# caidj0/Raytracer-2025

Hardware: AMD Instinct MI355X
Metric: Msamples/s (pixels x traced spp / s), book-1 random spheres 1920x1080, 512 spp (484 traced) (higher is better)
Workload: dtype f64

## Files before the change

### include/rt_mi355x.h

```cpp
#ifndef RT_MI355X_H
#define RT_MI355X_H

#include <stddef.h>
#include <stdint.h>

#ifdef __cplusplus
extern "C" {
#endif

#define RT_ABI_VERSION 3

enum rt_status {
    RT_OK = 0,
    RT_EINVAL = -1,
    RT_EHANDLE = -2,
    RT_EMOVED = -3,
    RT_EDEGENERATE = -4,
    RT_EPANIC = -5,
    RT_EUNSUPPORTED = -6,
    RT_EDEVICE = -7,
    RT_ENOMEM = -8,
    RT_ESTACK = -9
};

// ... 243 lines not shown
int32_t rt_render_gather_mode(const rt_scene* s);

int32_t rt_render_partials_get(rt_scene* s, double* out, uint64_t n_values);

int32_t rt_render_primary_get(rt_scene* s, uint16_t* out, uint64_t n_values);

int32_t rt_math_selftest(int32_t fn, int32_t impl, const double* a, const double* b, double* out, uint64_t n);

int32_t rt_walk_selftest(int32_t fn, const double* in, double* out, uint64_t n);

int32_t rt_disney_selftest(int32_t fn, const rt_disney_params* params, const double base_color[3], const double* in,
                           double* out, uint64_t n);

int32_t rt_bvh_selftest(rt_scene* s, int32_t list);
int32_t rt_world_selftest(rt_scene* s, int32_t world, int32_t lights, int32_t background_tex);

#define RT_COMM_ID_BYTES 128
int32_t rt_comm_unique_id(uint8_t id[RT_COMM_ID_BYTES]);
rt_comm* rt_comm_init(const uint8_t id[RT_COMM_ID_BYTES], int32_t nranks, int32_t rank);
void rt_comm_destroy(rt_comm* comm);

int32_t rt_to_rgb_device(const float* linear_device, uint8_t* srgb_device, uint64_t n_values, int32_t toon_map,
                         void* stream);
int32_t rt_write_png(const char* path, uint32_t width, uint32_t height, const uint8_t* rgb);
int32_t rt_camera_from_json(const char* path, rt_camera* cam);

#ifdef __cplusplus
}
#endif
#endif
// ... 1 lines not shown
```

### raytracer-2025_amd/capi.py

```python
import ctypes as C

c_double3 = C.c_double * 3
c_double4 = C.c_double * 4


class RtCamera(C.Structure):

    _fields_ = [
        ("aspect_ratio", C.c_double),
        ("image_width", C.c_uint32),
        ("samples_per_pixel", C.c_uint32),
        ("max_depth", C.c_uint32),
        ("background_tex", C.c_int32),
        ("vertical_fov_in_degrees", C.c_double),
        ("look_from", c_double3),
        ("look_at", c_double3),
        ("vec_up", c_double3),
        ("defocus_angle_in_degrees", C.c_double),
        ("focus_distance", C.c_double),
        ("toon_map", C.c_int32),
        ("reserved", C.c_int32),
    ]


# ... 227 lines not shown
    "shard_rows": (_U, [C.POINTER(RtCamera), C.POINTER(RtRenderOpts)]),
    "render_device": (_I, [_P, _I, _I, C.POINTER(RtCamera), C.POINTER(RtRenderOpts), _P]),
    "render_device_wait": (_I, [_P, C.POINTER(RtStats)]),
    "render_gather_mode": (_I, [_P]),
    "to_rgb_device": (_I, [_P, _P, C.c_uint64, _I, _P]),
    "write_png": (_I, [C.c_char_p, C.c_uint32, C.c_uint32, _P]),
    "camera_from_json": (_I, [C.c_char_p, C.POINTER(RtCamera)]),
    "world_info_get": (_I, [_P, _I, _I, _I, _U, C.POINTER(RtWorldInfo)]),
    "render_partials_get": (_I, [_P, _DP, C.c_uint64]),
    "render_primary_get": (_I, [_P, C.POINTER(C.c_uint16), C.c_uint64]),
    "math_selftest": (_I, [_I, _I, _DP, _DP, _DP, C.c_uint64]),
    "walk_selftest": (_I, [_I, _DP, _DP, C.c_uint64]),
    "disney_selftest": (_I, [_I, C.POINTER(RtDisneyParams), _DP, _DP, _DP, C.c_uint64]),
    "bvh_selftest": (_I, [_P, _I]),
    "world_selftest": (_I, [_P, _I, _I, _I]),
    "comm_unique_id": (_I, [C.POINTER(C.c_uint8)]),
    "comm_init": (_P, [C.POINTER(C.c_uint8), _I, _I]),
    "comm_destroy": (None, [_P]),
}

GPU_ONLY = ("world_hit", "world_hit_device", "world_occluded", "world_occluded_device", "radiance_opts_default", "world_radiance", "world_radiance_device", "lights_opts_default", "lights_pdf", "lights_pdf_device", "lights_sample", "lights_sample_device", "scatter_opts_default", "world_scatter", "world_scatter_device", "render_gather_mode", "render_partials_get", "render_primary_get", "math_selftest", "walk_selftest", "disney_params_default", "mat_disney", "mat_portal", "wavefront_load_flags", "disney_selftest", "bvh_selftest", "world_selftest", "comm_unique_id", "comm_init", "comm_destroy")

ORACLE_EXTRAS = {
    "render_partials": (_I, [_P, _I, _I, C.POINTER(RtCamera), C.POINTER(RtRenderOpts), _DP, C.POINTER(RtStats)]),
    "render_f64": (_I, [_P, _I, _I, C.POINTER(RtCamera), C.POINTER(RtRenderOpts), _DP, C.POINTER(C.c_uint8),
                        C.POINTER(RtStats), C.POINTER(C.c_uint64)]),
    "work_count_fields": (_U, []),
}

STATUS = {
    0: "RT_OK", -1: "RT_EINVAL", -2: "RT_EHANDLE", -3: "RT_EMOVED", -4: "RT_EDEGENERATE",
    -5: "RT_EPANIC", -6: "RT_EUNSUPPORTED", -7: "RT_EDEVICE", -8: "RT_ENOMEM", -9: "RT_ESTACK",
}


class RtError(RuntimeError):
# ... 37 lines not shown
```

### raytracer-2025_amd/csrc/rt_builds.h

```cpp
#pragma once
#include <hip/hip_runtime.h>

#include "rt_kernel.h"

namespace rtk {

struct Diag {
#ifdef RT_DIAG
    unsigned long long cyc_refill = 0, cyc_trace = 0, cyc_shade = 0, cyc_media = 0;
    unsigned long long cyc_miss = 0, cyc_queue = 0, cyc_draws = 0;
    unsigned long long wave_trace_iters = 0, lane_trace_iters = 0, node_visits = 0, sphere_tests = 0, main_iters = 0;
    unsigned long long load_cyc = 0, loads = 0;
    unsigned long long pops = 0, pop_reads = 0;
    unsigned long long big_tests = 0, big_hits = 0;
    unsigned long long u_steps = 0, u_uniform = 0, u_uniform_node = 0, u_active = 0, u_same = 0;
    unsigned long long u_top[4] = {0, 0, 0, 0}, l_top[4] = {0, 0, 0, 0}, l_node = 0;
    unsigned long long sh_rounds = 0, sh_lanes = 0, sh_classes = 0;
    unsigned long long pure_rounds = 0, pure_lanes = 0, pure_max_pn = 0;
    unsigned long long cls_rounds[11] = {}, cls_lanes[11] = {};
    unsigned long long cyc_camera = 0, prim_rays = 0, prim_tests = 0;
#endif
};
#ifdef RT_DIAG
constexpr int RT_DIAG_N = 64;
__device__ unsigned long long g_diag[RT_DIAG_N];
#define RT_DIAG_ONLY(x) x
#else
#define RT_DIAG_ONLY(x)
#endif
#ifdef RT_ISA_MARKS
#define RT_ISA_MARK(name) asm volatile(";@@phase " name)
#else
#define RT_ISA_MARK(name)
#endif

#ifdef RT_WAVE_TRACE
constexpr uint32_t RT_TRACE_LANES = 1u << 19, RT_TRACE_W = 12;
__device__ unsigned long long g_lane_trace[RT_TRACE_LANES * RT_TRACE_W];
constexpr uint32_t RT_HIST_N = 1024, RT_HIST_TICKS = 25000;
// ... 20 lines not shown
#ifdef RT_CHECK
constexpr uint32_t K_CHECK_SLAB = 15;
static_assert(K_CHECK_SLAB > K_POPXF, "the slab guard's marker must not be a ref kind");
constexpr uint32_t K_CHECK_PRIMARY = 14;
static_assert(K_CHECK_PRIMARY > K_POPXF, "the primary-ray guard's marker must not be a ref kind");
__device__ unsigned long long g_check[2];
__device__ __noinline__ void check_fail(uint32_t ref) {
    atomicAdd(&g_check[0], 1ull);
    atomicCAS(&g_check[1], 0ull, (1ull << 32) | ref);
}
#endif
__device__ __forceinline__ uint32_t ref_idx(const SceneView& S, uint32_t ref) {
    const uint32_t i = ref_index(ref);
#ifdef RT_CHECK
    const uint32_t k = ref_kind(ref);
    if (k != K_NONE && i >= S.n_ref[k]) {
        check_fail(ref);
        return 0u;
    }
#endif
    return i;
}
__device__ __forceinline__ void check_run(const SceneView& S, uint32_t first, uint32_t n) {
#ifdef RT_CHECK
    if (n && first + n > S.n_ref[K_QUAD]) check_fail(make_ref(K_QUAD, first + n - 1));
#endif
}

}
```

### raytracer-2025_amd/csrc/rt_kernel_hit.hip

```cpp
#include <hip/hip_runtime.h>

#include "../../include/rt_mi355x.h"
#include "rt_kernel.h"
#include "rt_math.h"
#include "rt_builds.h"
#include "rt_geom.h"
#include "rt_stack.h"
#include "rt_walk.h"
#include "rt_walk4.h"
#include "rt_record.h"

namespace rtk {

struct HitParams {
    SceneView S;
    const rt_ray* rays;
    rt_hit_record* out;
    uint64_t n;
    uint32_t key0, key1;
    RT_GLOBAL uint2* stack_ovf;
};

template <int TIER>
__global__ void __launch_bounds__(TIER == TIER_BASIC ? RT_BLOCK_BASIC : RT_BLOCK) rt_hit_kernel(const HitParams P) {
// ... 21 lines not shown
    for (uint64_t w0 = (uint64_t)blockIdx.x * BLK + (threadIdx.x & ~63u); w0 < P.n; w0 += stride) {
        const uint64_t i = w0 + (threadIdx.x & 63u);
        const bool live = i < P.n;
        Ray ray{};
        double t_max = 0.0;
        if (live) {
            const rt_ray q = P.rays[i];
            ray.o = d3(q.origin[0], q.origin[1], q.origin[2]);
            ray.d = d3(q.dir[0], q.dir[1], q.dir[2]);
            ray.time = q.time;
            t_max = q.t_max;
        }
        rng.pixel = (uint32_t)i;
        rng.begin(1);
        Trav<TIER> T;
        trace_begin<TIER>(S, ray, T);
        T.cl.set(t_max);
        if constexpr (B4) {
            if (!live) T.cur = 0u;
            bool walking = live;
            while (__ballot(walking))
                walking = trace4_step(S, ray, T, stk, pq, (const RT_LDS float4*)node_lds, dg);
        } else if (live) {
            while (trace_step<TIER>(S, ray, T, stk, rng, med, dg)) {
            }
            if constexpr (tier_full(TIER)) media_phase<TIER>(S, ray, T, stk, rng, med);
        }
        if (live) {
            rt_hit_record o{};
            o.mat = -1;
            if (T.found) {
                bool panic = false;
// ... 41 lines not shown
```

### raytracer-2025_amd/csrc/rt_kernel_occl.hip

```cpp
#include <hip/hip_runtime.h>

#include "../../include/rt_mi355x.h"
#include "rt_kernel.h"
#include "rt_math.h"
#include "rt_builds.h"
#include "rt_geom.h"
#include "rt_stack.h"
#include "rt_walk.h"
#include "rt_walk4.h"

namespace rtk {

struct OcclParams {
    SceneView S;
    const rt_ray* rays;
    uint8_t* out;
    uint64_t n;
    uint32_t key0, key1;
    RT_GLOBAL uint2* stack_ovf;
};

template <int TIER>
__global__ void __launch_bounds__(TIER == TIER_BASIC ? RT_BLOCK_BASIC : RT_BLOCK) rt_occl_kernel(const OcclParams P) {
    const SceneView& S = P.S;
// ... 20 lines not shown
    for (uint64_t w0 = (uint64_t)blockIdx.x * BLK + (threadIdx.x & ~63u); w0 < P.n; w0 += stride) {
        const uint64_t i = w0 + (threadIdx.x & 63u);
        const bool live = i < P.n;
        Ray ray{};
        double t_max = 0.0;
        if (live) {
            const rt_ray q = P.rays[i];
            ray.o = d3(q.origin[0], q.origin[1], q.origin[2]);
            ray.d = d3(q.dir[0], q.dir[1], q.dir[2]);
            ray.time = q.time;
            t_max = q.t_max;
        }
        rng.pixel = (uint32_t)i;
        rng.begin(1);
        Trav<TIER> T;
        trace_begin<TIER>(S, ray, T);
        T.cl.set(t_max);
        if constexpr (B4) {
            if (!live) T.cur = 0u;
            bool walking = live;
            while (__ballot(walking)) {
                walking = trace4_step(S, ray, T, stk, pq, (const RT_LDS float4*)node_lds, dg);
                if (T.found) {
                    T.cur = 0u;
                    T.sp = 0;
                    T.pn = 0;
                    walking = false;
                }
            }
        } else if (live) {
            while (!T.found && trace_step<TIER>(S, ray, T, stk, rng, med, dg)) {
            }
            if constexpr (tier_full(TIER)) {
                if (!T.found) media_phase<TIER>(S, ray, T, stk, rng, med);
            }
// ... 31 lines not shown
```

### raytracer-2025_amd/csrc/rt_kernel_path.hip

```cpp
#include <hip/hip_runtime.h>

#include "../../include/rt_mi355x.h"
#include "rt_kernel.h"
#include "rt_math.h"
#include "rt_slab.h"
#include "rt_primary.h"
#include "rt_plan.h"
#include "rt_queue.h"
#include "rt_path_entry.h"
#include "rt_builds.h"
#include "rt_frame.h"
#include "rt_texture.h"
#include "rt_geom.h"
#include "rt_stack.h"
#include "rt_walk.h"
#include "rt_walk4.h"
#include "rt_record.h"
#include "rt_lights.h"
#include "rt_shade.h"

namespace rtk {

#ifndef RT_BASIC_WAVES
#define RT_BASIC_WAVES 4
// ... 196 lines not shown
                if (!walking) {
                    T.cl.c = __builtin_huge_val();
                    T.cl.c_f = __builtin_huge_valf();
                    T.sp = 0;
                    T.found = false;
                    T.pn = 0;
                    T.nxf = 0;
                    T.hit.nxf = 0;
                    T.nmed = 0;
                    const bool begin = !no_path && !pmiss;
                    T.cur = begin ? bword(S, S.world_root) : 0u;
                    if (begin) {
                        rng.begin(vertex);
                        ++n_rays;
                        walking = true;
                    }
                } else {
                    trace_unpark_state2(T, pk2);
                }
            } else if (!no_path && !walking) {
                rng.begin(vertex);
                ++n_rays;
                trace_begin<TIER>(S, ray, T);
                walking = true;
            }
            RT_DIAG_ONLY(const unsigned long long t_b0 = __builtin_amdgcn_s_memtime(); dg.cyc_refill += t_b0 - t_loop0;)
            RT_ISA_MARK("walk");
            auto step = [&]() -> bool {
                return trace4_step(S, ray, T, stk, pq, (const RT_LDS float4*)node_lds, dg);
            };
            if constexpr (BATCH >= 64) {
#ifdef RT_WAVE_TRACE
                while (walking) walking = step(), ++trace_steps;
#else
                while (walking) walking = step();
#endif
            } else {
                const unsigned long long active = __ballot(true);
// ... 363 lines not shown
    atomicAdd(&g_diag[20], dg.u_same);
    for (int k = 0; k < 4; ++k) {
        atomicAdd(&g_diag[24 + k], dg.u_top[k]);
        atomicAdd(&g_diag[28 + k], dg.l_top[k]);
    }
    atomicAdd(&g_diag[32], dg.l_node);
    atomicAdd(&g_diag[33], dg.sh_rounds);
    atomicAdd(&g_diag[34], dg.sh_lanes);
    atomicAdd(&g_diag[35], dg.sh_classes);
    atomicAdd(&g_diag[36], dg.pure_rounds);
    atomicAdd(&g_diag[37], dg.pure_lanes);
    atomicAdd(&g_diag[38], dg.pure_max_pn);
    if (lane == 0) atomicAdd(&g_diag[61], dg.cyc_camera);
    atomicAdd(&g_diag[62], dg.prim_rays);
    atomicAdd(&g_diag[63], dg.prim_tests);
    for (int k = 0; k < 11; ++k) {
        atomicAdd(&g_diag[39 + k], dg.cls_rounds[k]);
        atomicAdd(&g_diag[50 + k], dg.cls_lanes[k]);
    }
#endif
#ifdef RT_WAVE_TRACE
    hist.flush();
    if (trace_lane < RT_TRACE_LANES) {
        unsigned long long* t = g_lane_trace + (uint64_t)trace_lane * RT_TRACE_W;
        t[0] = trace_t0;
        t[1] = __builtin_amdgcn_s_memrealtime();
        t[2] = trace_items;
        t[3] = n_rays;
        t[4] = trace_tq;
        t[5] = trace_q;
// ... 149 lines not shown
```

### raytracer-2025_amd/csrc/rt_kernel_radiance.hip

```cpp
#include <hip/hip_runtime.h>

#include "../../include/rt_mi355x.h"
#include "rt_kernel.h"
#include "rt_math.h"
#include "rt_queue.h"
#include "rt_builds.h"
#include "rt_texture.h"
#include "rt_geom.h"
#include "rt_stack.h"
#include "rt_walk.h"
#include "rt_walk4.h"
#include "rt_record.h"
#include "rt_lights.h"
#include "rt_shade.h"

namespace rtk {

struct RadParams {
    SceneView S;
    const rt_ray* rays;
    rt_radiance* out;
    uint32_t n;
    uint32_t first_index;
    uint32_t samples, max_depth;
// ... 99 lines not shown
        double t_max = 0.0;
        const bool first_walk = !done && !in_path;
        if (first_walk) {
            const rt_ray q = P.rays[item];
            ray.o = d3(q.origin[0], q.origin[1], q.origin[2]);
            ray.d = d3(q.dir[0], q.dir[1], q.dir[2]);
            ray.time = q.time;
            t_max = q.t_max;
            rng.sample = s;
            beta = d3(1, 1, 1);
            L = d3(0, 0, 0);
            vertex = 1;
            in_path = true;
        }
        Trav<TIER> T;
        trace_begin<TIER>(S, ray, T);
        if (in_path) {
            rng.begin(vertex);
            if (first_walk) T.cl.set(t_max);
        }
        if constexpr (B4) {
            if (!in_path) T.cur = 0u;
            bool walking = in_path;
            while (__ballot(walking))
                walking = trace4_step(S, ray, T, stk, pq, (const RT_LDS float4*)node_lds, dg);
        } else {
            while (trace_step<TIER>(S, ray, T, stk, rng, med, dg)) {
            }
            if constexpr (tier_full(TIER)) media_phase<TIER>(S, ray, T, stk, rng, med);
        }
        if (!in_path) continue;
        bool panic = false;
        bool end_path;
        if constexpr (B4) {
// ... 94 lines not shown
```

### raytracer-2025_amd/csrc/rt_kernel_scatter.hip

```cpp
#include <hip/hip_runtime.h>

#include "../../include/rt_mi355x.h"
#include "rt_kernel.h"
#include "rt_math.h"
#include "rt_builds.h"
#include "rt_texture.h"
#include "rt_geom.h"
#include "rt_stack.h"
#include "rt_walk.h"
#include "rt_walk4.h"
#include "rt_record.h"
#include "rt_lights.h"
#include "rt_shade.h"
#include "rt_scatter.h"

namespace rtk {

struct ScatterParams {
    SceneView S;
    const rt_ray* rays;
    const double* eval_dirs;
    const uint32_t* indices;
    rt_scatter* out;
    uint64_t n;
// ... 51 lines not shown
        const uint64_t i = w0 + (threadIdx.x & 63u);
        const bool live = i < P.n;
        Ray ray{};
        double t_max = 0.0;
        rng.pixel = P.first_index + (uint32_t)i;
        if (live) {
            const rt_ray q = P.rays[i];
            ray.o = d3(q.origin[0], q.origin[1], q.origin[2]);
            ray.d = d3(q.dir[0], q.dir[1], q.dir[2]);
            ray.time = q.time;
            t_max = q.t_max;
            if (P.indices) rng.pixel = P.indices[i];
        }
        rng.begin(P.vertex);
        Trav<TIER> T;
        trace_begin<TIER>(S, ray, T);
        T.cl.set(t_max);
        if constexpr (B4) {
            if (!live) T.cur = 0u;
            bool walking = live;
            while (__ballot(walking))
                walking = trace4_step(S, ray, T, stk, pq, (const RT_LDS float4*)node_lds, dg);
        } else if (live) {
            while (trace_step<TIER>(S, ray, T, stk, rng, med, dg)) {
            }
            if constexpr (tier_full(TIER)) media_phase<TIER>(S, ray, T, stk, rng, med);
        }
        if (!live) continue;
        char* const rec_out = (char*)&P.out[i];
        {
            double v[10] = {0, 0, 0, 0, 0, 0, 0, 0, 0, 0};
            int32_t mat = -1;
// ... 71 lines not shown
```

### raytracer-2025_amd/csrc/rt_layout.h

```cpp
#pragma once
#include "rt_planar_filter.h"
#include <hip/hip_runtime.h>
#include <stdint.h>

#if defined(__HIP_DEVICE_COMPILE__)
#define RT_GLOBAL __attribute__((address_space(1)))
#define RT_LDS __attribute__((address_space(3)))
#else
#define RT_GLOBAL
#define RT_LDS
#endif

namespace rtk {

enum RefKind : uint32_t {
    K_NONE = 0,
    K_BVH = 1,
    K_LIST = 2,
    K_SPHERE = 3,
    K_MSPHERE = 4,
    K_QUAD = 5,
    K_TRI = 6,
    K_XFORM = 7,
    K_MEDIUM = 8,
    K_POPXF = 9,
};

__host__ __device__ inline uint32_t make_ref(uint32_t kind, uint32_t index) { return (kind << 28) | index; }
__host__ __device__ inline uint32_t ref_kind(uint32_t r) { return r >> 28; }
__host__ __device__ inline uint32_t ref_index(uint32_t r) { return r & 0x0FFFFFFFu; }
constexpr uint32_t REF_NONE = 0u;

struct alignas(16) DNodeSlot {
    union {
        struct {
            float lo[3], hi[3];
            uint32_t pad[2];
        } box;
        double sphere[4];
    };
};
struct alignas(16) DNode {
    DNodeSlot slot[2];
    uint32_t c0, c1;
    uint32_t pad[2];
};
// ... 137 lines not shown
    const RT_GLOBAL DXform* xforms;
    const RT_GLOBAL DMedium* media;
    const RT_GLOBAL DMaterial* materials;
    const RT_GLOBAL DTexture* textures;
    const RT_GLOBAL float* texels;
    const RT_GLOBAL DPerlin* perlin;
    uint32_t world_root;
    uint32_t lights_root;
    int32_t background_tex;
    int32_t bg_kind;
    double bg_c0[3], bg_c1[3];
    uint32_t stack_need;
    uint32_t features;
    uint32_t n_nodes4;
    uint32_t n_perlin;
    uint32_t n_ref[16];
};

enum : int32_t { BG_NONE = 0, BG_SKY = 1, BG_OTHER = 2 };

enum : uint32_t {
    F_XFORM = 1u,
    F_MEDIUM = 2u,
    F_PLANAR = 4u,
    F_MSPHERE = 8u,
    F_LIGHTS = 16u,
    F_TEXFULL = 32u,
    F_MATFULL = 64u,
    F_REMAP = 128u,
    F_GENERAL = 512u,
    F_NORMALMAP = 256u,
    F_DISNEY = 1024u,
// ... 5 lines not shown
```

### raytracer-2025_amd/csrc/rt_render.cpp

```cpp
#include <dlfcn.h>

#include <algorithm>
#include <chrono>
#include <cstdlib>
#include <cstring>
#include <memory>
#include <mutex>
#include <map>
#include <thread>

#include <rccl/rccl.h>

#include "../../include/rt_mi355x.h"
#include "rt_kernel.h"
#include "rt_primary.h"
#include "rt_scene.hpp"

namespace {
struct RcclApi {
    bool ok = false;
    std::string err;
    ncclResult_t (*get_unique_id)(ncclUniqueId*) = nullptr;
    ncclResult_t (*comm_init_rank)(ncclComm_t*, int, ncclUniqueId, int) = nullptr;
    ncclResult_t (*comm_init_all)(ncclComm_t*, int, const int*) = nullptr;
// ... 224 lines not shown
        bvh4_convert(hw, RT_STACK_BASIC, true, rtk::NODE_LDS_CAP, rtk::NODE_LDS_CAP_BATCH) > RT_STACK_BASIC)
        tier = rtk::TIER_MESH;
    if (tier == rtk::TIER_MESH && bvh4_convert(hw, RT_STACK_MAX, false) > RT_STACK_MAX) tier = rtk::TIER_FULL;
    if (tier == rtk::TIER_FULL && hw.nodes.empty()) return rtk::TIER_FULL_FLAT;
    if (rtk::tier_full_bvh(tier)) {
        const uint32_t need = bvh4_convert(hw, RT_STACK_MAX, false);
        if (need > RT_STACK_MAX) {
            set_error(RT_ESTACK, "world needs " + std::to_string(need) + " traversal-stack entries, kernel has " +
                                     std::to_string(RT_STACK_MAX));
            return -1;
        }
    }
    return tier;
}

static int32_t hip_fail(hipError_t e, const char* what) {
    return set_error(RT_EDEVICE, std::string(what) + ": " + hipGetErrorString(e));
}

template <class T>
static size_t put(std::vector<char>& blob, const std::vector<T>& v) {
    size_t off = (blob.size() + 255) & ~(size_t)255;
    blob.resize(off + v.size() * sizeof(T));
    if (!v.empty()) std::memcpy(blob.data() + off, v.data(), v.size() * sizeof(T));
    return off;
}

static void pack_world(const HostWorld& hw, std::vector<char>& blob, rtk::SceneView& v) {
    auto off = [](size_t o) { return (uintptr_t)o; };
    v.portals = (const rtk::DPortal*)off(put(blob, hw.portals));
// ... 41 lines not shown
static int32_t build_flat(rt_scene* s, int32_t world, int32_t lights, int32_t bg, bool reference_bvh, FlatWorld& fw) {
    std::lock_guard<std::mutex> lk(fw.m);
    if (fw.done) {
        if (fw.rc != RT_OK) set_error(fw.rc, fw.err);
        return fw.rc;
    }
    fw.done = true;
    auto t0 = std::chrono::steady_clock::now();
    HostWorld hw;
    int32_t rc = flatten(s, world, lights, bg, reference_bvh, hw);
    constexpr uint32_t MATERIAL_TIERS = rtk::F_DISNEY | rtk::F_PORTAL | rtk::F_GENERAL;
    fw.has_disney = rc == RT_OK && (hw.features & MATERIAL_TIERS) != 0;
    if (fw.for_query) hw.features &= ~MATERIAL_TIERS;
    int tier = rc == RT_OK ? prepare_tier(hw) : -1;
    if (rc == RT_OK && tier < 0) rc = RT_ESTACK;
#ifdef RT_CHECK
    if (rc == RT_OK && std::getenv("RT_CHECK_INJECT") && std::getenv("RT_CHECK_INJECT")[0] == '1') {
        for (rtk::DNode4& nd : hw.nodes4)
            for (int k = 0; k < 4; ++k) {
                const uint32_t kind = rtk::ref_kind(nd.ref[k]);
                const size_t n = kind == rtk::K_SPHERE ? hw.spheres.size()
                                 : (kind == rtk::K_QUAD || kind == rtk::K_TRI) ? hw.planars.size() : 0;
                if (n) nd.ref[k] = rtk::make_ref(kind, (uint32_t)n + rtk::ref_index(nd.ref[k]));
            }
    }
#endif
    if (rc == RT_OK) {
        const uint32_t stack_cap = rtk_stack_entries(tier);
        if (hw.stack_need > stack_cap)
            rc = set_error(RT_ESTACK, "world needs " + std::to_string(hw.stack_need) +
// ... 19 lines not shown
            for (int k = 0; k < 3; ++k) v.bg_c0[k] = t.color[k], v.bg_c1[k] = t.color2[k];
    }
    v.stack_need = hw.stack_need;
    v.features = hw.features;
    v.n_nodes4 = (uint32_t)hw.nodes4.size();
    v.n_perlin = (uint32_t)hw.perlin.size();
    std::memset(v.n_ref, 0, sizeof v.n_ref);
    v.n_ref[rtk::K_BVH] = (uint32_t)hw.nodes4.size();
    v.n_ref[rtk::K_LIST] = (uint32_t)hw.list_children.size();
    v.n_ref[rtk::K_SPHERE] = (uint32_t)hw.spheres.size();
    v.n_ref[rtk::K_MSPHERE] = (uint32_t)hw.msph_center.size();
    v.n_ref[rtk::K_QUAD] = v.n_ref[rtk::K_TRI] = (uint32_t)hw.planars.size();
    v.n_ref[rtk::K_XFORM] = (uint32_t)hw.xforms.size();
    v.n_ref[rtk::K_MEDIUM] = (uint32_t)hw.media.size();
    v.n_ref[rtk::K_POPXF] = 1;
    fw.tier = tier;
    fw.stack_need = hw.stack_need;
    fw.n_prims = hw.n_prims;
    fw.ms = std::chrono::duration<double, std::milli>(std::chrono::steady_clock::now() - t0).count();
    return RT_OK;
}

static int32_t slot_for(RenderState* r, size_t k, int device, DeviceWorld*& out) {
    DeviceWorld* d = r->slots[k];
    if (d && d->device != device) {
        destroy_device_world(d);
        r->slots[k] = d = nullptr;
        (void)hipSetDevice(device);
    }
    if (d) {
// ... 1078 lines not shown
    return lights_device(s, world, lights, opts, L_SAMPLE, origins3_dev, nullptr, n, out_dev);
}

int32_t rt_world_info_get(rt_scene* s, int32_t world, int32_t lights, int32_t bg, uint32_t flags, rt_world_info* out) {
    if (!s || !out) return set_error(RT_EINVAL, "null argument");
    if (world < 0 || (size_t)world >= s->objs.size() || s->objs[world].hidden)
        return set_error(RT_EHANDLE, "unknown world handle");
    try {
        HostWorld hw;
        int32_t rc = flatten(s, world, lights, bg, (flags & RT_FLAG_REFERENCE_BVH) != 0, hw);
        if (rc != RT_OK) return rc;
        out->primitives = (uint32_t)hw.n_prims;
        out->bvh_leaves = (uint32_t)hw.n_bvh_leaves;
        const int tier = prepare_tier(hw);
        if (tier < 0) return RT_ESTACK;
        std::vector<char> blob;
        rtk::SceneView view{};
        pack_world(hw, blob, view);
        out->device_bytes = blob.size();
        out->bvh_nodes = (uint32_t)hw.nodes4.size();
        out->stack_need = hw.stack_need;
        out->kernel_tier = (uint32_t)tier;
        out->features = hw.features;
        return RT_OK;
    } catch (const std::bad_alloc&) {
        return set_error(RT_ENOMEM, "out of host memory");
    }
}

int32_t rt_render_device_wait(rt_scene* s, rt_stats* st) {
    return wait(s, st);
}

int32_t rt_render_gather_mode(const rt_scene* s) {
    const RenderState* r = s ? s->rs : nullptr;
    if (!r || r->n_parts == 0) return set_error(RT_EINVAL, "nothing rendered on this scene");
    return r->gather_mode;
}

// ... 231 lines not shown
```

### raytracer-2025_amd/csrc/rt_scene.cpp

```cpp
#include "rt_kernel.h"
#include "rt_image.hpp"
#include "rt_scene.hpp"
#include "rt_slab.h"

#include <algorithm>
#include <cstring>
#include <exception>
#include <functional>
#include <limits>
#include <system_error>
#include <thread>
#include <unordered_map>

#include "../../include/rt_mi355x.h"

#ifndef RT_EXPAND_LEAF_LISTS
#define RT_EXPAND_LEAF_LISTS 1
#endif

namespace rth {

static thread_local std::string g_error;
int32_t set_error(int32_t code, const std::string& msg) {
    g_error = msg;
// ... 194 lines not shown
constexpr int MAX_XF_NESTING = 2;

#ifndef RT_SAH_SWEEP_MAX
#define RT_SAH_SWEEP_MAX 2048
#endif

struct Flattener {
    const rt_scene* s;
    HostWorld& out;
    bool reference_bvh;
    std::unordered_map<int, std::pair<uint32_t, uint32_t>> memo;
    bool no_collapse = false;
    std::unordered_map<int, Box3> tight_memo;
    std::string err;
    int32_t code = RT_OK;
    static constexpr uint32_t REF_NONE_ = rtk::REF_NONE;

    uint32_t fail(int32_t c, const std::string& m) {
        if (code == RT_OK) {
            code = c;
            err = m;
        }
        return REF_NONE_;
    }

    Box3 tight(int id) {
        const Obj& o = s->objs[id];
        if (o.kind != O_LIST && o.kind != O_BVH && o.kind != O_XFORM && o.kind != O_MEDIUM) return o.bbox;
        if (o.kind == O_BVH && o.hidden) {
            Box3 b = Box3::empty();
// ... 59 lines not shown
            const double4 sp = out.spheres[rtk::ref_index(ref)];
            n.slot[which].sphere[0] = sp.x;
            n.slot[which].sphere[1] = sp.y;
            n.slot[which].sphere[2] = sp.z;
            n.slot[which].sphere[3] = sp.w;
        }
        else
            set_box(n, which, b);
    }

    struct Item {
        uint32_t ref, need;
        Box3 box;
        double c[3];
    };

    struct NodeBuf {
        std::vector<rtk::DNode> n;
        std::vector<uint8_t> local;
        uint32_t splice(const NodeBuf& sub) {
            const uint32_t off = (uint32_t)n.size();
            n.insert(n.end(), sub.n.begin(), sub.n.end());
            local.insert(local.end(), sub.local.begin(), sub.local.end());
            for (size_t k = off; k < n.size(); ++k) {
                if (local[k] & 1u) n[k].c0 += off;
                if (local[k] & 2u) n[k].c1 += off;
            }
            return off;
        }
    };
// ... 333 lines not shown
                if (!reference_bvh && !no_collapse && o.children.size() >= 2 &&
                    std::any_of(o.children.begin(), o.children.end(), [&](int c) { return holds_bvh(c, 0); })) {
                    std::vector<int> elems;
                    for (int c : o.children) list_elements(c, elems, 0);
                    std::vector<Item> items;
                    for (int c : elems) {
                        auto e = emit(c, in_boundary, xf_depth);
                        Item x;
                        x.ref = e.first;
                        x.need = e.second;
                        x.box = tight(c);
                        for (int k = 0; k < 3; ++k) x.c[k] = 0.5 * (x.box.a[k].lo + x.box.a[k].hi);
                        items.push_back(x);
                    }
                    out.n_bvh_leaves += items.size();
                    r = sah(items, 0, items.size());
                    break;
                }
                std::vector<std::pair<uint32_t, uint32_t>> kids;
                for (int c : o.children) kids.push_back(emit(c, in_boundary, xf_depth));
                uint32_t start = (uint32_t)out.list_children.size();
                for (size_t i = 0; i < kids.size(); ++i) {
                    out.list_children.push_back(kids[i].first);
                    out.list_boxes.push_back(boxf(tight(o.children[i])));
                }
                out.list_children.push_back(REF_NONE_);
                out.list_boxes.push_back(boxf(Box3::empty()));
                uint32_t need = 0;
                for (size_t i = 0; i < kids.size(); ++i) {
                    bool last = i + 1 == kids.size();
// ... 9 lines not shown
                }
                std::vector<int> leaves;
                collect_leaves(id, leaves);
                std::vector<Item> items;
                items.reserve(leaves.size());
                for (int l : leaves) {
                    auto e = emit(l, in_boundary, xf_depth);
                    Item x;
                    x.ref = e.first;
                    x.need = e.second;
                    x.box = tight(l);
                    for (int k = 0; k < 3; ++k) x.c[k] = 0.5 * (x.box.a[k].lo + x.box.a[k].hi);
                    items.push_back(x);
                }
                out.n_bvh_leaves += items.size();
                if (items.size() == 1) {
                    uint32_t idx = (uint32_t)out.nodes.size();
                    out.nodes.emplace_back();
                    rtk::DNode& n = out.nodes[idx];
                    set_child(n, 0, items[0].ref, items[0].box);
                    set_box(n, 1, Box3::empty());
                    n.c0 = items[0].ref;
                    n.c1 = REF_NONE_;
                    r = {rtk::make_ref(rtk::K_BVH, idx), std::max<uint32_t>(1, items[0].need)};
                } else {
                    r = sah(items, 0, items.size());
                }
                break;
            }
            case O_XFORM: {
// ... 84 lines not shown
static int tex_needs_uv(const rt_scene* s, int t, int depth = 0) {
    if (t < 0 || depth > 16) return 0;
    const TexRec& r = s->texs[t];
    if (r.type == rtk::T_IMAGE) return r.h != 0;
    if (r.type == rtk::T_CHECKER) return tex_needs_uv(s, r.even, depth + 1) | tex_needs_uv(s, r.odd, depth + 1);
    return 0;
}

int32_t lights_check(const rt_scene* s, int32_t lights) {
    std::string lerr;
    const int lk = light_tree(s, lights, 0, lerr);
    return lk < 0 ? set_error(lk, lerr) : RT_OK;
}

int32_t flatten(const rt_scene* s, int32_t world, int32_t lights, int32_t background_tex, bool reference_bvh,
                HostWorld& out) {
    out = HostWorld();
    for (size_t i = 0; i < s->texs.size(); ++i) {
        const TexRec& r = s->texs[i];
        rtk::DTexture t{};
        t.type = r.type;
        for (int k = 0; k < 3; ++k) {
            t.color[k] = r.color[k];
            t.color2[k] = r.color2[k];
        }
        t.scale = r.scale;
        t.a = r.type == rtk::T_CHECKER ? r.even : (int32_t)r.w;
        t.b = r.type == rtk::T_CHECKER ? r.odd : (int32_t)r.h;
        t.c = r.linear;
        t.data = r.type == rtk::T_IMAGE ? r.texel_offset : (uint64_t)(r.perlin < 0 ? 0 : r.perlin);
        t.needs_uv = tex_needs_uv(s, (int)i);
// ... 24 lines not shown
            for (int k = 0; k < 3; ++k) m.albedo[k] = s->texs[m.tex].color[k];
        }
        m.flags = f;
    }
    for (int pass = 0; pass < 4; ++pass)
        for (size_t i = 0; i < out.materials.size(); ++i) {
            rtk::DMaterial& m = out.materials[i];
            if (m.type == rtk::M_DIFFUSE_LIGHT || m.type == rtk::M_MIX) {
                for (int sub : {m.inner, m.inner2})
                    if (sub >= 0) m.flags |= out.materials[sub].flags & (rtk::MF_NEEDS_UV | rtk::MF_EMISSIVE);
            }
        }
    if (background_tex >= (int32_t)s->texs.size()) return set_error(RT_EHANDLE, "unknown background texture");

    Flattener F{s, out, reference_bvh, {}, false, {}, {}, RT_OK};
    auto W = F.emit(world, false, 0);
    if (F.code != RT_OK) return set_error(F.code, F.err);
    out.world_root = W.first;
    out.stack_need = 1 + W.second;
    out.lights_root = rtk::REF_NONE;
    if (lights >= 0) {
        std::string lerr;
        const int lk = light_tree(s, lights, 0, lerr);
        if (lk < 0) return set_error(lk, lerr);
        if (lk == 2) out.features |= rtk::F_GENERAL;
        F.no_collapse = true;
        F.memo.erase(lights);
        auto Lr = F.emit(lights, false, 0);
        F.no_collapse = false;
        if (F.code != RT_OK) return set_error(F.code, F.err);
// ... 456 lines not shown
        for (size_t i = s->objs.size(); i < a.objs.size(); ++i) {
            const Obj &x = a.objs[i], &y = b.objs[i];
            if (x.kind != y.kind || x.left != y.left || x.right != y.right || x.hidden != y.hidden ||
                std::memcmp(&x.bbox, &y.bbox, sizeof(Box3)) != 0)
                return 0;
        }
        return 1;
    } catch (const std::bad_alloc&) {
        return set_error(RT_ENOMEM, "out of host memory");
    }
}
int32_t rt_world_selftest(rt_scene* s, int32_t world, int32_t lights, int32_t background_tex) {
    if (!s) return set_error(RT_EINVAL, "null argument");
    try {
        HostWorld p, q;
        int32_t rc = flatten(s, world, lights, background_tex, false, p);
        if (rc != RT_OK) return rc;
        g_serial_build = true;
        rc = flatten(s, world, lights, background_tex, false, q);
        g_serial_build = false;
        if (rc != RT_OK) return rc;
        auto same = [](const auto& x, const auto& y) {
            return x.size() == y.size() && (x.empty() || std::memcmp(x.data(), y.data(), x.size() * sizeof(x[0])) == 0);
        };
        return (same(p.nodes, q.nodes) && same(p.list_children, q.list_children) && same(p.planars, q.planars) &&
                same(p.spheres, q.spheres) && p.world_root == q.world_root && p.lights_root == q.lights_root &&
                p.stack_need == q.stack_need)
                   ? 1
                   : 0;
    } catch (const std::bad_alloc&) {
        g_serial_build = false;
        return set_error(RT_ENOMEM, "out of host memory");
    }
}
int32_t rt_build_box(rt_scene* s, const double a[3], const double b[3], int32_t mat) {
    if (!s || bad(a) || bad(b)) return set_error(RT_EINVAL, "null argument");
    if (!mat_ok(s, mat)) return set_error(RT_EHANDLE, "unknown material");
    V3 mn(std::fmin(a[0], b[0]), std::fmin(a[1], b[1]), std::fmin(a[2], b[2]));
    V3 mx(std::fmax(a[0], b[0]), std::fmax(a[1], b[1]), std::fmax(a[2], b[2]));
    V3 dx(mx.x - mn.x, 0, 0), dy(0, mx.y - mn.y, 0), dz(0, 0, mx.z - mn.z);
    int32_t list = rt_hittables_new(s);
// ... 430 lines not shown
```

### raytracer-2025_amd/csrc/rt_scene.hpp

```cpp
#pragma once
#include <cmath>
#include <cstdint>
#include <memory>
#include <string>
#include <vector>

#include "rt_layout.h"

namespace rth {

struct V3 {
    double x = 0, y = 0, z = 0;
    V3() = default;
    V3(double a, double b, double c) : x(a), y(b), z(c) {}
    explicit V3(const double* p) : x(p[0]), y(p[1]), z(p[2]) {}
    double operator[](int i) const { return i == 0 ? x : (i == 1 ? y : z); }
};
inline V3 operator+(V3 a, V3 b) { return V3(a.x + b.x, a.y + b.y, a.z + b.z); }
inline V3 operator-(V3 a, V3 b) { return V3(a.x - b.x, a.y - b.y, a.z - b.z); }
inline V3 operator*(V3 a, V3 b) { return V3(a.x * b.x, a.y * b.y, a.z * b.z); }
inline V3 operator/(V3 a, V3 b) { return V3(a.x / b.x, a.y / b.y, a.z / b.z); }
inline V3 operator*(double s, V3 v) { return V3(s * v.x, s * v.y, s * v.z); }
inline V3 operator-(V3 a) { return V3(-a.x, -a.y, -a.z); }
inline double dot(V3 a, V3 b) { return a.x * b.x + a.y * b.y + a.z * b.z; }
// ... 83 lines not shown
    std::vector<uint32_t> list_children;
    std::vector<rtk::DBoxF> list_boxes;
    std::vector<rtk::DXform> xforms;
    std::vector<rtk::DMedium> media;
    std::vector<rtk::DMaterial> materials;
    std::vector<rtk::DTexture> textures;
    std::vector<float> texels;
    std::vector<rtk::DPerlin> perlin;
    std::vector<rtk::DDisney> disney;
    std::vector<rtk::DPortal> portals;
    uint32_t world_root = 0, lights_root = 0;
    uint32_t stack_need = 0;
    uint32_t features = 0;
    size_t n_prims = 0;
    size_t n_bvh_leaves = 0;
};

struct RenderState;

}

struct rt_scene {
    std::vector<rth::Obj> objs;
    std::vector<rth::TexRec> texs;
    std::vector<rth::MatRec> mats;
    std::vector<float> texels;
    std::vector<rtk::DPerlin> perlins;
    std::vector<rtk::DDisney> disneys;
    std::vector<rtk::DPortal> portals;
    uint32_t next_medium_id = 0;
    uint64_t generation = 0;
    rth::RenderState* rs = nullptr;
};

namespace rth {
int32_t set_error(int32_t code, const std::string& msg);
int32_t flatten(const rt_scene* s, int32_t world, int32_t lights, int32_t background_tex, bool reference_bvh,
                HostWorld& out);
int32_t lights_check(const rt_scene* s, int32_t lights);
uint32_t bvh4_convert(HostWorld& hw, uint32_t max_need, bool filter_spheres, size_t max_nodes = SIZE_MAX,
                      size_t variant_nodes = 0);
void destroy_render_state(RenderState* r);
}
```

### raytracer-2025_amd/csrc/rt_walk.h

```cpp
#pragma once
#include "rt_builds.h"
#include "rt_geom.h"
#include "rt_kernel.h"
#include "rt_math.h"
#include "rt_slab.h"
#include "rt_stack.h"

namespace rtk {

constexpr float NO_CULL = -__builtin_huge_valf();
template <int TIER>
constexpr bool flat_boxes() { return TIER == TIER_FULL_FLAT; }
template <int TIER>
constexpr bool unified_load() {
    return TIER == TIER_MESH || tier_full_bvh(TIER);
}
__device__ __forceinline__ double f4_lo(float4 q) { return __hiloint2double(__float_as_int(q.y), __float_as_int(q.x)); }
__device__ __forceinline__ double f4_hi(float4 q) { return __hiloint2double(__float_as_int(q.w), __float_as_int(q.z)); }
template <int TIER>
constexpr bool flat_runs() { return TIER == TIER_FULL_FLAT; }

__device__ __forceinline__ bool list_box_hit(const SceneView& S, uint32_t li, const RayF& rf, float tmin_f,
                                             float c_f) {
    const RT_GLOBAL float4* bp = reinterpret_cast<const RT_GLOBAL float4*>(S.list_boxes + li);
// ... 193 lines not shown
    bool found;
    HitInfo hit;
    uint32_t nmed;
    uint32_t pn;
    static_assert(RT_SLAB_FOLD == 1, "the basic tier's sign-ordered slab test (RaySF) needs RT_SLAB_FOLD = 1");
    RaySF sf;
    uint32_t so[3];
};
__device__ __forceinline__ void trace_sorted_fields(const Ray& wr, Trav<TIER_BASIC>& T) {
    const double o[3] = {wr.o.x, wr.o.y, wr.o.z}, d[3] = {wr.d.x, wr.d.y, wr.d.z};
    T.sf = make_raysf(o, d);
#pragma unroll
    for (int k = 0; k < 3; ++k) T.so[k] = T.sf.pos[k] ? 0u : 3u * (uint32_t)sizeof(float4);
}

template <int TIER>
__device__ __forceinline__ void trace_begin(const SceneView& S, const Ray& wr, Trav<TIER>& T) {
    T.r = wr;
    T.rf = make_rayf(wr);
    T.a = len2(wr.d);
    T.inva = 1.0 / T.a;
    T.cl.c = __builtin_huge_val();
    T.cl.c_f = __builtin_huge_valf();
    T.cur = S.world_root;
    T.sp = 0;
    T.nxf = 0;
    T.found = false;
    T.hit.nxf = 0;
    T.nmed = 0;
    if constexpr (TIER == TIER_BASIC) {
        T.pn = 0;
        T.cur = bword(S, S.world_root);
        trace_sorted_fields(wr, T);
    }
}

template <class Park>
__device__ __forceinline__ void trace_park(const Trav<TIER_MESH>& T, Park pk) {
    constexpr uint32_t B = RT_BLOCK;
    const uint64_t c = (uint64_t)__double_as_longlong(T.cl.c), ht = (uint64_t)__double_as_longlong(T.hit.t);
    pk[0 * B] = T.cur;
    pk[1 * B] = T.sp | ((uint32_t)T.found << 16);
    pk[2 * B] = (uint32_t)c;
    pk[3 * B] = (uint32_t)(c >> 32);
    pk[4 * B] = __float_as_uint(T.cl.c_f);
    pk[5 * B] = (uint32_t)ht;
    pk[6 * B] = (uint32_t)(ht >> 32);
    pk[7 * B] = T.hit.ref;
// ... 304 lines not shown
```

Measured before the change: 9349.

## Hoist huge ground spheres out of the BVH and test them first

At build time, spheres in the top-level BVH whose bounding box covers at least half the scene's surface area (up to two) are removed from the BVH and recorded in the scene view. At the start of each basic-tier traversal those spheres are intersected directly, which sets an early closest-hit bound and gives a tighter BVH for the remaining primitives. The huge ground sphere in the random-spheres scene otherwise inflates every BVH node box and causes many wasted node visits. The cost is two extra sphere tests per ray, plus a second flatten pass on the host at setup.

```diff
diff --git a/include/rt_mi355x.h b/include/rt_mi355x.h
--- a/include/rt_mi355x.h
+++ b/include/rt_mi355x.h
@@ -281,6 +281,7 @@
 
 int32_t rt_bvh_selftest(rt_scene* s, int32_t list);
 int32_t rt_world_selftest(rt_scene* s, int32_t world, int32_t lights, int32_t background_tex);
+int32_t rt_world_hoisted_get(rt_scene* s, int32_t world, uint32_t flags, uint32_t* idx, uint32_t cap);
 
 #define RT_COMM_ID_BYTES 128
 int32_t rt_comm_unique_id(uint8_t id[RT_COMM_ID_BYTES]);
diff --git a/raytracer-2025_amd/capi.py b/raytracer-2025_amd/capi.py
--- a/raytracer-2025_amd/capi.py
+++ b/raytracer-2025_amd/capi.py
@@ -265,12 +265,13 @@
     "disney_selftest": (_I, [_I, C.POINTER(RtDisneyParams), _DP, _DP, _DP, C.c_uint64]),
     "bvh_selftest": (_I, [_P, _I]),
     "world_selftest": (_I, [_P, _I, _I, _I]),
+    "world_hoisted_get": (_I, [_P, _I, _U, C.POINTER(C.c_uint32), _U]),
     "comm_unique_id": (_I, [C.POINTER(C.c_uint8)]),
     "comm_init": (_P, [C.POINTER(C.c_uint8), _I, _I]),
     "comm_destroy": (None, [_P]),
 }
 
-GPU_ONLY = ("world_hit", "world_hit_device", "world_occluded", "world_occluded_device", "radiance_opts_default", "world_radiance", "world_radiance_device", "lights_opts_default", "lights_pdf", "lights_pdf_device", "lights_sample", "lights_sample_device", "scatter_opts_default", "world_scatter", "world_scatter_device", "render_gather_mode", "render_partials_get", "render_primary_get", "math_selftest", "walk_selftest", "disney_params_default", "mat_disney", "mat_portal", "wavefront_load_flags", "disney_selftest", "bvh_selftest", "world_selftest", "comm_unique_id", "comm_init", "comm_destroy")
+GPU_ONLY = ("world_hit", "world_hit_device", "world_occluded", "world_occluded_device", "radiance_opts_default", "world_radiance", "world_radiance_device", "lights_opts_default", "lights_pdf", "lights_pdf_device", "lights_sample", "lights_sample_device", "scatter_opts_default", "world_scatter", "world_scatter_device", "render_gather_mode", "render_partials_get", "render_primary_get", "math_selftest", "walk_selftest", "disney_params_default", "mat_disney", "mat_portal", "wavefront_load_flags", "disney_selftest", "bvh_selftest", "world_selftest", "world_hoisted_get", "comm_unique_id", "comm_init", "comm_destroy")
 
 ORACLE_EXTRAS = {
     "render_partials": (_I, [_P, _I, _I, C.POINTER(RtCamera), C.POINTER(RtRenderOpts), _DP, C.POINTER(RtStats)]),
diff --git a/raytracer-2025_amd/csrc/rt_builds.h b/raytracer-2025_amd/csrc/rt_builds.h
--- a/raytracer-2025_amd/csrc/rt_builds.h
+++ b/raytracer-2025_amd/csrc/rt_builds.h
@@ -19,10 +19,11 @@
     unsigned long long pure_rounds = 0, pure_lanes = 0, pure_max_pn = 0;
     unsigned long long cls_rounds[11] = {}, cls_lanes[11] = {};
     unsigned long long cyc_camera = 0, prim_rays = 0, prim_tests = 0;
+    unsigned long long hoist_tests = 0, hoist_hits = 0;
 #endif
 };
 #ifdef RT_DIAG
-constexpr int RT_DIAG_N = 64;
+constexpr int RT_DIAG_N = 66;
 __device__ unsigned long long g_diag[RT_DIAG_N];
 #define RT_DIAG_ONLY(x) x
 #else
@@ -73,7 +74,7 @@
     const uint32_t i = ref_index(ref);
 #ifdef RT_CHECK
     const uint32_t k = ref_kind(ref);
-    if (k != K_NONE && i >= S.n_ref[k]) {
+    if (k != K_NONE && (k >= RT_REF_KINDS || i >= S.n_ref[k])) {
         check_fail(ref);
         return 0u;
     }
diff --git a/raytracer-2025_amd/csrc/rt_kernel_hit.hip b/raytracer-2025_amd/csrc/rt_kernel_hit.hip
--- a/raytracer-2025_amd/csrc/rt_kernel_hit.hip
+++ b/raytracer-2025_amd/csrc/rt_kernel_hit.hip
@@ -59,8 +59,8 @@
         rng.pixel = (uint32_t)i;
         rng.begin(1);
         Trav<TIER> T;
-        trace_begin<TIER>(S, ray, T);
-        T.cl.set(t_max);
+        trace_begin<TIER>(S, ray, T, t_max);
+        if constexpr (!B4) T.cl.set(t_max);
         if constexpr (B4) {
             if (!live) T.cur = 0u;
             bool walking = live;
diff --git a/raytracer-2025_amd/csrc/rt_kernel_occl.hip b/raytracer-2025_amd/csrc/rt_kernel_occl.hip
--- a/raytracer-2025_amd/csrc/rt_kernel_occl.hip
+++ b/raytracer-2025_amd/csrc/rt_kernel_occl.hip
@@ -58,11 +58,11 @@
         rng.pixel = (uint32_t)i;
         rng.begin(1);
         Trav<TIER> T;
-        trace_begin<TIER>(S, ray, T);
-        T.cl.set(t_max);
+        trace_begin<TIER>(S, ray, T, t_max);
+        if constexpr (!B4) T.cl.set(t_max);
         if constexpr (B4) {
-            if (!live) T.cur = 0u;
-            bool walking = live;
+            if (!live || T.found) T.cur = 0u;
+            bool walking = live && !T.found;
             while (__ballot(walking)) {
                 walking = trace4_step(S, ray, T, stk, pq, (const RT_LDS float4*)node_lds, dg);
                 if (T.found) {
diff --git a/raytracer-2025_amd/csrc/rt_kernel_path.hip b/raytracer-2025_amd/csrc/rt_kernel_path.hip
--- a/raytracer-2025_amd/csrc/rt_kernel_path.hip
+++ b/raytracer-2025_amd/csrc/rt_kernel_path.hip
@@ -234,6 +234,7 @@
                         rng.begin(vertex);
                         ++n_rays;
                         walking = true;
+                        hoist_test(S, ray, T, &dg);
                     }
                 } else {
                     trace_unpark_state2(T, pk2);
@@ -241,7 +242,7 @@
             } else if (!no_path && !walking) {
                 rng.begin(vertex);
                 ++n_rays;
-                trace_begin<TIER>(S, ray, T);
+                trace_begin<TIER>(S, ray, T, __builtin_huge_val(), &dg);
                 walking = true;
             }
             RT_DIAG_ONLY(const unsigned long long t_b0 = __builtin_amdgcn_s_memtime(); dg.cyc_refill += t_b0 - t_loop0;)
@@ -635,6 +636,8 @@
     if (lane == 0) atomicAdd(&g_diag[61], dg.cyc_camera);
     atomicAdd(&g_diag[62], dg.prim_rays);
     atomicAdd(&g_diag[63], dg.prim_tests);
+    atomicAdd(&g_diag[64], dg.hoist_tests);
+    atomicAdd(&g_diag[65], dg.hoist_hits);
     for (int k = 0; k < 11; ++k) {
         atomicAdd(&g_diag[39 + k], dg.cls_rounds[k]);
         atomicAdd(&g_diag[50 + k], dg.cls_lanes[k]);
diff --git a/raytracer-2025_amd/csrc/rt_kernel_radiance.hip b/raytracer-2025_amd/csrc/rt_kernel_radiance.hip
--- a/raytracer-2025_amd/csrc/rt_kernel_radiance.hip
+++ b/raytracer-2025_amd/csrc/rt_kernel_radiance.hip
@@ -137,10 +137,11 @@
             in_path = true;
         }
         Trav<TIER> T;
-        trace_begin<TIER>(S, ray, T);
+        trace_begin<TIER>(S, ray, T, in_path && first_walk ? t_max : __builtin_huge_val());
         if (in_path) {
             rng.begin(vertex);
-            if (first_walk) T.cl.set(t_max);
+            if constexpr (!B4)
+                if (first_walk) T.cl.set(t_max);
         }
         if constexpr (B4) {
             if (!in_path) T.cur = 0u;
diff --git a/raytracer-2025_amd/csrc/rt_kernel_scatter.hip b/raytracer-2025_amd/csrc/rt_kernel_scatter.hip
--- a/raytracer-2025_amd/csrc/rt_kernel_scatter.hip
+++ b/raytracer-2025_amd/csrc/rt_kernel_scatter.hip
@@ -89,8 +89,8 @@
         }
         rng.begin(P.vertex);
         Trav<TIER> T;
-        trace_begin<TIER>(S, ray, T);
-        T.cl.set(t_max);
+        trace_begin<TIER>(S, ray, T, t_max);
+        if constexpr (!B4) T.cl.set(t_max);
         if constexpr (B4) {
             if (!live) T.cur = 0u;
             bool walking = live;
diff --git a/raytracer-2025_amd/csrc/rt_layout.h b/raytracer-2025_amd/csrc/rt_layout.h
--- a/raytracer-2025_amd/csrc/rt_layout.h
+++ b/raytracer-2025_amd/csrc/rt_layout.h
@@ -30,6 +30,8 @@
 __host__ __device__ inline uint32_t ref_kind(uint32_t r) { return r >> 28; }
 __host__ __device__ inline uint32_t ref_index(uint32_t r) { return r & 0x0FFFFFFFu; }
 constexpr uint32_t REF_NONE = 0u;
+constexpr uint32_t RT_REF_KINDS = 12;
+#define RT_HOIST_MAX 2
 
 struct alignas(16) DNodeSlot {
     union {
@@ -197,8 +199,12 @@
     uint32_t features;
     uint32_t n_nodes4;
     uint32_t n_perlin;
-    uint32_t n_ref[16];
-};
+    uint32_t n_ref[RT_REF_KINDS];
+    uint32_t n_hoist;
+    uint32_t hoist[RT_HOIST_MAX];
+    uint32_t hoist_pad;
+};
+static_assert(RT_REF_KINDS + 2 + RT_HOIST_MAX == 16, "n_ref and the hoist fields fill n_ref's former 16 words");
 
 enum : int32_t { BG_NONE = 0, BG_SKY = 1, BG_OTHER = 2 };
 
diff --git a/raytracer-2025_amd/csrc/rt_render.cpp b/raytracer-2025_amd/csrc/rt_render.cpp
--- a/raytracer-2025_amd/csrc/rt_render.cpp
+++ b/raytracer-2025_amd/csrc/rt_render.cpp
@@ -262,6 +262,17 @@
     return tier;
 }
 
+static void hoist_basic(const rt_scene* s, int32_t world, int32_t lights, int32_t bg, bool reference_bvh, uint32_t drop,
+                        HostWorld& hw) {
+    if (reference_bvh || hw.nodes4.empty()) return;
+    HostWorld h2;
+    if (flatten(s, world, lights, bg, false, h2, true) != RT_OK || h2.hoisted.empty()) return;
+    h2.features &= ~drop;
+    if (prepare_tier(h2) != rtk::TIER_BASIC) return;
+    if ((h2.nodes4.size() > rtk::NODE_LDS_CAP_BATCH) != (hw.nodes4.size() > rtk::NODE_LDS_CAP_BATCH)) return;
+    hw = std::move(h2);
+}
+
 static int32_t hip_fail(hipError_t e, const char* what) {
     return set_error(RT_EDEVICE, std::string(what) + ": " + hipGetErrorString(e));
 }
@@ -333,6 +344,8 @@
     if (fw.for_query) hw.features &= ~MATERIAL_TIERS;
     int tier = rc == RT_OK ? prepare_tier(hw) : -1;
     if (rc == RT_OK && tier < 0) rc = RT_ESTACK;
+    if (tier == rtk::TIER_BASIC)
+        hoist_basic(s, world, lights, bg, reference_bvh, fw.for_query ? MATERIAL_TIERS : 0u, hw);
 #ifdef RT_CHECK
     if (rc == RT_OK && std::getenv("RT_CHECK_INJECT") && std::getenv("RT_CHECK_INJECT")[0] == '1') {
         for (rtk::DNode4& nd : hw.nodes4)
@@ -382,6 +395,9 @@
     v.n_ref[rtk::K_XFORM] = (uint32_t)hw.xforms.size();
     v.n_ref[rtk::K_MEDIUM] = (uint32_t)hw.media.size();
     v.n_ref[rtk::K_POPXF] = 1;
+    v.n_hoist = (uint32_t)hw.hoisted.size();
+    for (uint32_t k = 0; k < RT_HOIST_MAX; ++k) v.hoist[k] = k < v.n_hoist ? hw.hoisted[k] : 0u;
+    v.hoist_pad = 0;
     fw.tier = tier;
     fw.stack_need = hw.stack_need;
     fw.n_prims = hw.n_prims;
@@ -1490,6 +1506,8 @@
         out->bvh_leaves = (uint32_t)hw.n_bvh_leaves;
         const int tier = prepare_tier(hw);
         if (tier < 0) return RT_ESTACK;
+        if (tier == rtk::TIER_BASIC)
+            hoist_basic(s, world, lights, bg, (flags & RT_FLAG_REFERENCE_BVH) != 0, 0u, hw);
         std::vector<char> blob;
         rtk::SceneView view{};
         pack_world(hw, blob, view);
@@ -1499,6 +1517,26 @@
         out->kernel_tier = (uint32_t)tier;
         out->features = hw.features;
         return RT_OK;
+    } catch (const std::bad_alloc&) {
+        return set_error(RT_ENOMEM, "out of host memory");
+    }
+}
+
+int32_t rt_world_hoisted_get(rt_scene* s, int32_t world, uint32_t flags, uint32_t* idx, uint32_t cap) {
+    if (!s || (cap && !idx)) return set_error(RT_EINVAL, "null argument");
+    if (flags & ~RT_FLAG_REFERENCE_BVH) return set_error(RT_EINVAL, "unknown flags");
+    if (world < 0 || (size_t)world >= s->objs.size() || s->objs[world].hidden)
+        return set_error(RT_EHANDLE, "unknown world handle");
+    try {
+        HostWorld hw;
+        const bool reference_bvh = (flags & RT_FLAG_REFERENCE_BVH) != 0;
+        int32_t rc = flatten(s, world, -1, -1, reference_bvh, hw);
+        if (rc != RT_OK) return rc;
+        const int tier = prepare_tier(hw);
+        if (tier < 0) return RT_ESTACK;
+        if (tier == rtk::TIER_BASIC) hoist_basic(s, world, -1, -1, reference_bvh, 0u, hw);
+        for (uint32_t k = 0; k < cap && k < hw.hoisted.size(); ++k) idx[k] = hw.hoisted[k];
+        return (int32_t)hw.hoisted.size();
     } catch (const std::bad_alloc&) {
         return set_error(RT_ENOMEM, "out of host memory");
     }
diff --git a/raytracer-2025_amd/csrc/rt_scene.cpp b/raytracer-2025_amd/csrc/rt_scene.cpp
--- a/raytracer-2025_amd/csrc/rt_scene.cpp
+++ b/raytracer-2025_amd/csrc/rt_scene.cpp
@@ -232,6 +232,7 @@
     std::unordered_map<int, Box3> tight_memo;
     std::string err;
     int32_t code = RT_OK;
+    int hoist_id = -1;
     static constexpr uint32_t REF_NONE_ = rtk::REF_NONE;
 
     uint32_t fail(int32_t c, const std::string& m) {
@@ -321,6 +322,33 @@
         Box3 box;
         double c[3];
     };
+
+    static double half_area_f(const Box3& b) {
+        const rtk::DBoxF f = boxf(b);
+        const double dx = std::fmax((double)f.hi[0] - (double)f.lo[0], 0.0),
+                     dy = std::fmax((double)f.hi[1] - (double)f.lo[1], 0.0),
+                     dz = std::fmax((double)f.hi[2] - (double)f.lo[2], 0.0);
+        return dx * dy + dy * dz + dz * dx;
+    }
+    void pick_hoist(std::vector<Item>& items) {
+        Box3 all = Box3::empty();
+        for (const Item& x : items) all = all.unite(x.box);
+        const double whole = half_area_f(all);
+        std::vector<std::pair<double, uint32_t>> cand;
+        for (const Item& x : items)
+            if (rtk::ref_kind(x.ref) == rtk::K_SPHERE) {
+                const double a = half_area_f(x.box);
+                if (a >= 0.5 * whole) cand.push_back({-a, rtk::ref_index(x.ref)});
+            }
+        std::sort(cand.begin(), cand.end());
+        size_t n = std::min<size_t>(cand.size(), RT_HOIST_MAX);
+        if (n >= items.size()) n = items.size() - 1;
+        for (size_t k = 0; k < n; ++k) {
+            const uint32_t ref = rtk::make_ref(rtk::K_SPHERE, cand[k].second);
+            out.hoisted.push_back(cand[k].second);
+            items.erase(std::find_if(items.begin(), items.end(), [&](const Item& x) { return x.ref == ref; }));
+        }
+    }
 
     struct NodeBuf {
         std::vector<rtk::DNode> n;
@@ -684,6 +712,7 @@
                         items.push_back(x);
                     }
                     out.n_bvh_leaves += items.size();
+                    if (id == hoist_id) pick_hoist(items);
                     r = sah(items, 0, items.size());
                     break;
                 }
@@ -723,6 +752,7 @@
                     items.push_back(x);
                 }
                 out.n_bvh_leaves += items.size();
+                if (id == hoist_id) pick_hoist(items);
                 if (items.size() == 1) {
                     uint32_t idx = (uint32_t)out.nodes.size();
                     out.nodes.emplace_back();
@@ -837,7 +867,7 @@
 }
 
 int32_t flatten(const rt_scene* s, int32_t world, int32_t lights, int32_t background_tex, bool reference_bvh,
-                HostWorld& out) {
+                HostWorld& out, bool hoist) {
     out = HostWorld();
     for (size_t i = 0; i < s->texs.size(); ++i) {
         const TexRec& r = s->texs[i];
@@ -892,6 +922,16 @@
     if (background_tex >= (int32_t)s->texs.size()) return set_error(RT_EHANDLE, "unknown background texture");
 
     Flattener F{s, out, reference_bvh, {}, false, {}, {}, RT_OK};
+    if (hoist && !reference_bvh) {
+        int id = world;
+        for (int depth = 0; depth < 8 && s->objs[id].kind == O_LIST && s->objs[id].children.size() == 1; ++depth)
+            id = s->objs[id].children[0];
+        const Obj& o = s->objs[id];
+        if (o.kind == O_BVH ||
+            (o.kind == O_LIST && o.children.size() >= 2 &&
+             std::any_of(o.children.begin(), o.children.end(), [&](int c) { return F.holds_bvh(c, 0); })))
+            F.hoist_id = id;
+    }
     auto W = F.emit(world, false, 0);
     if (F.code != RT_OK) return set_error(F.code, F.err);
     out.world_root = W.first;
@@ -1378,17 +1418,17 @@
     if (!s) return set_error(RT_EINVAL, "null argument");
     try {
         HostWorld p, q;
-        int32_t rc = flatten(s, world, lights, background_tex, false, p);
+        int32_t rc = flatten(s, world, lights, background_tex, false, p, true);
         if (rc != RT_OK) return rc;
         g_serial_build = true;
-        rc = flatten(s, world, lights, background_tex, false, q);
+        rc = flatten(s, world, lights, background_tex, false, q, true);
         g_serial_build = false;
         if (rc != RT_OK) return rc;
         auto same = [](const auto& x, const auto& y) {
             return x.size() == y.size() && (x.empty() || std::memcmp(x.data(), y.data(), x.size() * sizeof(x[0])) == 0);
         };
         return (same(p.nodes, q.nodes) && same(p.list_children, q.list_children) && same(p.planars, q.planars) &&
-                same(p.spheres, q.spheres) && p.world_root == q.world_root && p.lights_root == q.lights_root &&
+                same(p.spheres, q.spheres) && same(p.hoisted, q.hoisted) && p.world_root == q.world_root && p.lights_root == q.lights_root &&
                 p.stack_need == q.stack_need)
                    ? 1
                    : 0;
diff --git a/raytracer-2025_amd/csrc/rt_scene.hpp b/raytracer-2025_amd/csrc/rt_scene.hpp
--- a/raytracer-2025_amd/csrc/rt_scene.hpp
+++ b/raytracer-2025_amd/csrc/rt_scene.hpp
@@ -121,6 +121,7 @@
     uint32_t features = 0;
     size_t n_prims = 0;
     size_t n_bvh_leaves = 0;
+    std::vector<uint32_t> hoisted;
 };
 
 struct RenderState;
@@ -143,7 +144,7 @@
 namespace rth {
 int32_t set_error(int32_t code, const std::string& msg);
 int32_t flatten(const rt_scene* s, int32_t world, int32_t lights, int32_t background_tex, bool reference_bvh,
-                HostWorld& out);
+                HostWorld& out, bool hoist = false);
 int32_t lights_check(const rt_scene* s, int32_t lights);
 uint32_t bvh4_convert(HostWorld& hw, uint32_t max_need, bool filter_spheres, size_t max_nodes = SIZE_MAX,
                       size_t variant_nodes = 0);
diff --git a/raytracer-2025_amd/csrc/rt_walk.h b/raytracer-2025_amd/csrc/rt_walk.h
--- a/raytracer-2025_amd/csrc/rt_walk.h
+++ b/raytracer-2025_amd/csrc/rt_walk.h
@@ -231,8 +231,34 @@
     for (int k = 0; k < 3; ++k) T.so[k] = T.sf.pos[k] ? 0u : 3u * (uint32_t)sizeof(float4);
 }
 
-template <int TIER>
-__device__ __forceinline__ void trace_begin(const SceneView& S, const Ray& wr, Trav<TIER>& T) {
+__device__ __forceinline__ void hoist_test(const SceneView& S, const Ray& r, Trav<TIER_BASIC>& T, Diag* dg) {
+#pragma unroll
+    for (uint32_t k = 0; k < RT_HOIST_MAX; ++k) {
+        if (k < S.n_hoist) {
+            const uint32_t idx = S.hoist[k];
+#if defined(__HIP_DEVICE_COMPILE__)
+            typedef const __attribute__((address_space(4))) double* ConstD;
+            ConstD sp = (ConstD)((uint64_t)S.spheres + (uint64_t)idx * sizeof(double4));
+#else
+            const double* sp = (const double*)(S.spheres + idx);
+#endif
+            const double cx = sp[0], cy = sp[1], cz = sp[2], rad = sp[3];
+            RT_DIAG_ONLY(if (dg)++ dg->hoist_tests;)
+            double t;
+            if (sphere_t_inv(d3(cx, cy, cz), rad, r, T.a, T.inva, 1e-8, T.cl.c, t)) {
+                RT_DIAG_ONLY(if (dg)++ dg->hoist_hits;)
+                T.cl.lower(t);
+                T.found = true;
+                T.hit.t = t;
+                T.hit.ref = make_ref(K_SPHERE, idx);
+            }
+        }
+    }
+}
+
+template <int TIER>
+__device__ __forceinline__ void trace_begin(const SceneView& S, const Ray& wr, Trav<TIER>& T,
+                                            double tmax = __builtin_huge_val(), Diag* dg = nullptr) {
     T.r = wr;
     T.rf = make_rayf(wr);
     T.a = len2(wr.d);
@@ -249,6 +275,8 @@
         T.pn = 0;
         T.cur = bword(S, S.world_root);
         trace_sorted_fields(wr, T);
+        T.cl.set(tmax);
+        hoist_test(S, wr, T, dg);
     }
 }
 
```

After: 9321. About the same (-0.3%).
